# GeoStat-Framework/PyKrige

Measured on AMD Instinct MI355X. Metric: kriged grid-points/sec (z + sigma^2), OK2D N=5000 on 1000x1000 grid, higher is better.
Workload: dtype f64

## Files before the change

### include/mikrige.h

```cpp
#ifndef MIKRIGE_H
#define MIKRIGE_H
#include <stdint.h>
#ifdef __cplusplus
extern "C" {
#endif

#define MIK_ABI_VERSION 9

#define MIK_OK          0
#define MIK_EINVAL     (-1)
#define MIK_ESINGULAR  (-2)
#define MIK_EHIP       (-3)
#define MIK_ERCCL      (-4)
#define MIK_ESTATE     (-5)

#define MIK_MODEL_LINEAR      0
#define MIK_MODEL_POWER       1
#define MIK_MODEL_GAUSSIAN    2
#define MIK_MODEL_SPHERICAL   3
#define MIK_MODEL_EXPONENTIAL 4
#define MIK_MODEL_HOLE_EFFECT 5
#define MIK_MODEL_CUSTOM      6

typedef struct mik_handle mik_handle;
// ... 58 lines not shown
  int32_t mw_kernel;
  int32_t half_sweep;
  int32_t factor_attempts;
  int32_t null_dim;
  int32_t rhs_overlapped;
  double verify_ms;
  double verify_res_z;
  double verify_res_inv;
  int32_t sparse;
  int32_t stations_sorted;
  double sparse_tiles;
  double sparse_tiles_dense;
  double sparse_ktiles;
  double sparse_ktiles_dense;
  double sparse_lists_ms;
  double sparse_diag_products;
  int32_t sparse_rows;
  int32_t points_sorted;
  double sort_points_ms;
  int32_t sparse_ktile;
  int32_t reserved2;
  double exchange_bytes;
} mik_timing;

int  mik_device_count(void);
int  mik_abi_version(void);
int  mik_create(int device, mik_handle **out);
void mik_destroy(mik_handle *h);

int  mik_set_devices(int n);
int  mik_handle_set_devices(mik_handle *h, int n);
int  mik_handle_devices(mik_handle *h);
int  mik_slab_of(int64_t n, int members, int i, int64_t *lo, int64_t *count);

int  mik_set_option(mik_handle *h, const char *key, double value);

typedef void (*mik_variogram_fn)(void *user, double *d_inout, int64_t rows, int64_t cols, int64_t ld);
int  mik_set_custom_variogram(mik_handle *h, mik_variogram_fn fn, void *user);

int  mik_set_problem(mik_handle *h, const mik_problem *p);
int  mik_station_order(const mik_problem *p, int32_t *order_out);
int  mik_factor(mik_handle *h);
int  mik_set_points(mik_handle *h, const mik_points *g);
int  mik_set_grid(mik_handle *h, const mik_grid *g);
int  mik_adjust_points(mik_handle *h, const double center[3], const double rot[9], const double stretch[3]);
int  mik_predict(mik_handle *h);
int  mik_get_results(mik_handle *h, double *z_out, double *ss_out);
int  mik_take_results(mik_handle *h, double **z, double **ss);
void mik_release_results(double *z);

int  mik_set_fields(mik_handle *h, const double *values, int64_t n, int32_t nf);
int  mik_get_field_results(mik_handle *h, double *z_out);

int  mik_set_field_gaps(mik_handle *h, const uint8_t *valid , int64_t n, int32_t nf);
int  mik_get_field_sigmasq(mik_handle *h, double *ss_out);
int  mik_synchronize(mik_handle *h);

int  mik_predict_moving_window(mik_handle *h, int n_closest_points);

int  mik_cross_validate(mik_handle *h, int n_closest_points , double *zhat_out , double *ss_out );

int  mik_cross_validate_folds(mik_handle *h, const int32_t *fold , int nfolds, double *zhat_out , double *ss_out );

int  mik_cross_validate_window(mik_handle *h, int n_closest_points, double *zhat_out , double *ss_out );

int  mik_predict_cov(mik_handle *h, double *cov_out );
// ... 39 lines not shown
```

### pykrige_amd/_lib.py

```python
import ctypes as C
import os

import numpy as np

_HERE = os.path.dirname(os.path.abspath(__file__))
LIB_PATH = os.environ.get("MIK_LIB_PATH") or os.path.join(_HERE, "libmikrige.so")

MIK_OK, MIK_EINVAL, MIK_ESINGULAR, MIK_EHIP, MIK_ERCCL, MIK_ESTATE = 0, -1, -2, -3, -4, -5
MODEL_IDS = {"linear": 0, "power": 1, "gaussian": 2, "spherical": 3, "exponential": 4, "hole-effect": 5, "custom": 6}
VARIOGRAM_FN = C.CFUNCTYPE(None, C.c_void_p, C.POINTER(C.c_double), C.c_int64, C.c_int64, C.c_int64)

_dp = C.POINTER(C.c_double)


class MikProblem(C.Structure):
    _fields_ = [
        ("ndim", C.c_int32), ("model_id", C.c_int32), ("n", C.c_int64),
        ("xs", _dp), ("ys", _dp), ("zs", _dp), ("values", _dp),
        ("params", C.c_double * 3), ("eps", C.c_double),
        ("exact_values", C.c_int32), ("regional_linear", C.c_int32), ("n_wells", C.c_int32), ("n_extra", C.c_int32),
        ("wells", _dp), ("extra_cols", _dp), ("a_inv", _dp),
        ("geographic", C.c_int32), ("pseudo_inv", C.c_int32),
    ]

# ... 19 lines not shown
    _fields_ = [
        ("assemble_ms", C.c_double), ("invert_ms", C.c_double), ("rhs_ms", C.c_double),
        ("contract_ms", C.c_double), ("predict_ms", C.c_double), ("contract_launches", C.c_int64),
        ("contract_flops_executed", C.c_double), ("factor_path", C.c_int32), ("symmetric", C.c_int32),
        ("engine", C.c_int32), ("reserved", C.c_int32),
        ("exchange_ms", C.c_double), ("exchange_path", C.c_int32), ("n_devices", C.c_int32),
        ("exchange_wait_ms", C.c_double), ("exchange_fallbacks", C.c_int32), ("rccl_ranks", C.c_int32),
        ("mw_kernel", C.c_int32), ("half_sweep", C.c_int32), ("factor_attempts", C.c_int32), ("null_dim", C.c_int32), ("rhs_overlapped", C.c_int32),
        ("verify_ms", C.c_double), ("verify_res_z", C.c_double), ("verify_res_inv", C.c_double),
        ("sparse", C.c_int32), ("stations_sorted", C.c_int32),
        ("sparse_tiles", C.c_double), ("sparse_tiles_dense", C.c_double),
        ("sparse_ktiles", C.c_double), ("sparse_ktiles_dense", C.c_double), ("sparse_lists_ms", C.c_double),
        ("sparse_diag_products", C.c_double), ("sparse_rows", C.c_int32), ("points_sorted", C.c_int32),
        ("sort_points_ms", C.c_double), ("sparse_ktile", C.c_int32), ("reserved2", C.c_int32), ("exchange_bytes", C.c_double),
    ]

    def as_dict(self):
        return {k: getattr(self, k) for k, _ in self._fields_}


_lib = None
ABI_VERSION = 9
CV_FOLDS_LDS = 96

SIGNATURES = {
    "mik_device_count": (C.c_int, []),
    "mik_abi_version": (C.c_int, []),
    "mik_create": (C.c_int, [C.c_int, C.POINTER(C.c_void_p)]),
    "mik_destroy": (None, [C.c_void_p]),
    "mik_set_devices": (C.c_int, [C.c_int]),
    "mik_handle_set_devices": (C.c_int, [C.c_void_p, C.c_int]),
    "mik_handle_devices": (C.c_int, [C.c_void_p]),
    "mik_slab_of": (C.c_int, [C.c_int64, C.c_int, C.c_int, C.POINTER(C.c_int64), C.POINTER(C.c_int64)]),
    "mik_get_device_timing": (C.c_int, [C.c_void_p, C.c_int, C.POINTER(MikTiming)]),
    "mik_set_option": (C.c_int, [C.c_void_p, C.c_char_p, C.c_double]),
    "mik_set_problem": (C.c_int, [C.c_void_p, C.POINTER(MikProblem)]),
    "mik_station_order": (C.c_int, [C.POINTER(MikProblem), C.POINTER(C.c_int32)]),
    "mik_factor": (C.c_int, [C.c_void_p]),
    "mik_set_points": (C.c_int, [C.c_void_p, C.POINTER(MikPoints)]),
    "mik_set_grid": (C.c_int, [C.c_void_p, C.POINTER(MikGrid)]),
    "mik_adjust_points": (C.c_int, [C.c_void_p, _dp, _dp, _dp]),
    "mik_predict": (C.c_int, [C.c_void_p]),
    "mik_get_results": (C.c_int, [C.c_void_p, _dp, _dp]),
    "mik_take_results": (C.c_int, [C.c_void_p, C.POINTER(_dp), C.POINTER(_dp)]),
    "mik_release_results": (None, [_dp]),
    "mik_set_fields": (C.c_int, [C.c_void_p, _dp, C.c_int64, C.c_int32]),
    "mik_get_field_results": (C.c_int, [C.c_void_p, _dp]),
    "mik_set_field_gaps": (C.c_int, [C.c_void_p, C.POINTER(C.c_uint8), C.c_int64, C.c_int32]),
    "mik_get_field_sigmasq": (C.c_int, [C.c_void_p, _dp]),
    "mik_synchronize": (C.c_int, [C.c_void_p]),
    "mik_set_custom_variogram": (C.c_int, [C.c_void_p, VARIOGRAM_FN, C.c_void_p]),
    "mik_predict_cov": (C.c_int, [C.c_void_p, _dp]),
    "mik_predict_block": (C.c_int, [C.c_void_p, _dp, C.c_int]),
    "mik_predict_block_window": (C.c_int, [C.c_void_p, _dp, C.c_int, C.c_int]),
    "mik_predict_moving_window": (C.c_int, [C.c_void_p, C.c_int]),
    "mik_predict_window_gaps": (C.c_int, [C.c_void_p, C.c_int, C.POINTER(C.c_uint8), _dp, _dp]),
    "mik_cross_validate": (C.c_int, [C.c_void_p, C.c_int, _dp, _dp]),
    "mik_cross_validate_folds": (C.c_int, [C.c_void_p, C.POINTER(C.c_int32), C.c_int, _dp, _dp]),
    "mik_cross_validate_window": (C.c_int, [C.c_void_p, C.c_int, _dp, _dp]),
    "mik_statistics": (C.c_int, [C.c_void_p, _dp, _dp]),
    "mik_experimental_variogram": (C.c_int, [C.c_void_p, C.c_int, _dp, _dp, C.POINTER(C.c_int32)]),
    "mik_krige_execute": (C.c_int, [C.c_int, C.POINTER(MikProblem), C.POINTER(MikPoints), _dp, _dp]),
    "mik_assemble_only": (C.c_int, [C.c_void_p]),
    "mik_get_matrix": (C.c_int, [C.c_void_p, C.c_int, _dp]),
    "mik_matrix_order": (C.c_int64, [C.c_void_p]),
    "mik_points_resident": (C.c_int64, [C.c_void_p]),
# ... 390 lines not shown
        self.option_epoch += 1
        check(self._lib.mik_comm_init(self._h, int(nranks), int(rank), C.create_string_buffer(uid, 128)))

    def bcast_factor(self, root=0):
        check(self._lib.mik_bcast_factor(self._h, int(root)))

    def factor_checksum(self):
        out = (C.c_uint64 * 4)()
        check(self._lib.mik_factor_checksum(self._h, out))
        return tuple(int(v) for v in out)

    def exchange_note(self):
        return (self._lib.mik_exchange_note(self._h) or b"").decode("utf-8", "replace")


def station_order(xs, ys, zs=None, geographic=False):
    xs, ys = _f64(xs), _f64(ys)
    zs = _f64(zs) if zs is not None else None
    p = MikProblem()
    p.ndim, p.n = (3 if zs is not None else 2), xs.size
    p.geographic = 1 if geographic else 0
    p.xs, p.ys, p.zs = _ptr(xs), _ptr(ys), _ptr(zs)
    out = np.zeros(xs.size, dtype=np.int32)
    check(load().mik_station_order(C.byref(p), out.ctypes.data_as(C.POINTER(C.c_int32))))
    return out


def slab_of(n, members, i):
    lo, cnt = C.c_int64(0), C.c_int64(0)
    check(load().mik_slab_of(int(n), int(members), int(i), C.byref(lo), C.byref(cnt)))
    return lo.value, cnt.value


def set_devices(n):
    flush_handle_pool()
    check(load().mik_set_devices(int(n)))


import threading as _threading

_pool_lock = _threading.Lock()
_pool = []


def _env_sig():
    return tuple(sorted((k, v) for k, v in os.environ.items() if k.startswith("MIK_") or k == "LOCAL_RANK"))


def acquire_handle():
    sig, pid = _env_sig(), os.getpid()
    with _pool_lock:
        for i, h in enumerate(_pool):
            if h.pid == pid and h.env_sig == sig:
                return _pool.pop(i)
    return Handle()


def release_handle(h, device_bytes):
    if h is None or not getattr(h, "_h", None):
        return
    try:
        limit = int(os.environ.get("MIK_HANDLE_POOL", "4"))
        cap = float(os.environ.get("MIK_HANDLE_POOL_BYTES", str(512 * 2 ** 20)))
    except ValueError:
        limit, cap = 0, 0.0
    if limit > 0 and h.option_epoch == 0 and getattr(h, "_custom_cb", None) is None and h.pid == os.getpid() and device_bytes <= cap:
# ... 39 lines not shown
```

### pykrige_amd/csrc/mik_host.h

```cpp
#pragma once
#include "mik_dev.h"
#include "../../include/mikrige.h"

#include <dlfcn.h>
#include <rccl/rccl.h>

#include <algorithm>
#include <array>
#include <cmath>
#include <cstdio>
#include <cstdlib>
#include <cstring>
#include <atomic>
#include <chrono>
#include <condition_variable>
#include <memory>
#include <map>
#include <mutex>
#include <string>
#include <thread>
#include <vector>

using namespace mik;

// ... 100 lines not shown
inline void host_copy(void* dst, const void* src, size_t bytes) {
  constexpr size_t PIECE = 8u << 20;
  const size_t nthr = std::min<size_t>(4, bytes / PIECE);
  if (nthr < 2) {
    memcpy(dst, src, bytes);
    return;
  }
  std::vector<std::thread> th;
  const size_t per = ((bytes / nthr + 63) / 64) * 64;
  for (size_t t = 1; t < nthr; ++t) {
    const size_t off = t * per, len = (t + 1 == nthr) ? bytes - off : per;
    th.emplace_back([=] { memcpy((char*)dst + off, (const char*)src + off, len); });
  }
  memcpy(dst, src, per);
  for (auto& t : th) t.join();
}

extern "C++" {
template <class F>
inline void parallel_chunks(long n, F fn) {
  const long nthr = std::min<long>(8, n / (1L << 20));
  if (nthr < 2) {
    fn(0, 0L, n);
    return;
  }
  std::vector<std::thread> th;
  const long per = (n + nthr - 1) / nthr;
  for (long t = 1; t < nthr; ++t) th.emplace_back([=] { fn((int)t, t * per, std::min(n, (t + 1) * per)); });
  fn(0, 0L, std::min(n, per));
  for (auto& t : th) t.join();
}
}
inline int chunks_of(long n) { return (int)std::max<long>(1, std::min<long>(8, n / (1L << 20))); }

inline void unmasked_positions(const int8_t* mask, long ncells, std::vector<long>& idx) {
  const int nc = chunks_of(ncells);
  std::vector<long> cnt(nc + 1, 0);
  parallel_chunks(ncells, [&](int c, long b, long e) {
    long k = 0;
    for (long i = b; i < e; ++i) k += mask[i] == 0;
    cnt[c + 1] = k;
  });
  for (int c = 0; c < nc; ++c) cnt[c + 1] += cnt[c];
  idx.resize((size_t)cnt[nc]);
  parallel_chunks(ncells, [&](int c, long b, long e) {
    long k = cnt[c];
    for (long i = b; i < e; ++i)
      if (!mask[i]) idx[(size_t)k++] = i;
  });
}

struct RcclApi {
  void* lib = nullptr;
  ncclResult_t (*GetUniqueId)(ncclUniqueId*) = nullptr;
  ncclResult_t (*CommInitRank)(ncclComm_t*, int, ncclUniqueId, int) = nullptr;
  ncclResult_t (*Broadcast)(const void*, void*, size_t, ncclDataType_t, int, ncclComm_t, hipStream_t) = nullptr;
  ncclResult_t (*CommDestroy)(ncclComm_t) = nullptr;
  const char* (*GetErrorString)(ncclResult_t) = nullptr;
  ncclResult_t (*CommInitAll)(ncclComm_t*, int, const int*) = nullptr;
  ncclResult_t (*GroupStart)() = nullptr;
  ncclResult_t (*GroupEnd)() = nullptr;
};
inline RcclApi g_rccl;
inline int rccl_load() {
  if (g_rccl.lib) return MIK_OK;
  const char* names[] = {getenv("MIK_RCCL_LIB") ? getenv("MIK_RCCL_LIB") : "librccl.so", "librccl.so", "librccl.so.1", "/opt/rocm/lib/librccl.so"};
// ... 102 lines not shown
  DevBuf Averify, vbuf;
  std::vector<double> hvals;
  int nf = 0;
  std::vector<double> hfields;
  DevBuf fv, fc, zf;
  PinBuf pin_fz;
  int fv_sorted = -1;
  int nf_done = 0;
  std::vector<uint8_t> hgaps;
  bool gaps_any = false;
  DevBuf gap_W, gap_work, gap_list, gap_part, gap_ss;
  PinBuf pin_gss;
  std::vector<int> gap_plane;
  PinBuf pin_cov;
  hipEvent_t ev_cov[6] = {nullptr, nullptr, nullptr, nullptr, nullptr, nullptr};
  int opt_gate = -1;
  int opt_panel_stream = -1;
  int opt_update_rev = -1;
  long npt_total = 0, npt = 0;
  bool masked = false;
  std::vector<long> scatter;
  const unsigned* scatter32 = nullptr;
  DevBuf mask_dev, mask_cnt;
  PinBuf scatter_pin;
  DevBuf px, py, pz, extra_rows, z, ss;
  DevBuf grid_axes, grid_idx;
  DevBuf mw_idx, mw_dist, stat_S, stat_x, stat_out;
  DevBuf cvw;
  int n_cu = 256;
  int t_state = 0;
  int opt_tri = 1;
  int opt_symmetrize = 1;
  int opt_factor = 0, opt_sym = 1;
  long opt_chunk = 131072;
  int opt_mw_pivot = 0;
  bool mw_force_piv = false;
  int opt_mw_lds_cap = 8192;
  int opt_mw_knn_bound = 1;
  int opt_mw_static = 1;
  int opt_mw_knn_lane = 1;
  int opt_mw_class = 0;
  mik_timing tm{};
  std::vector<hipEvent_t> evpool;
  std::vector<LaunchEvents> pr_launch;
  hipEvent_t ev_predict0 = nullptr, ev_predict1 = nullptr;
  hipEvent_t ev_lane1 = nullptr;
  hipEvent_t ev_sort = nullptr;
  hipEvent_t ev_chunk = nullptr;
  ncclComm_t comm = nullptr;
  int nranks = 1, rank = 0;
  PinBuf pin_in, pin_out;
  hipStream_t stream_d2h = nullptr;
  hipEvent_t ev_d2h = nullptr;
  bool results_on_host = false;
  long out_off = 0;
  std::vector<mik_handle*> kids;
  bool is_kid = false;
  bool alias_ok = false;
  int opt_exchange = 0;
  int exchange_used = 0;
  double exchange_ms = 0.0;
  std::string exchange_note;
  std::vector<std::vector<hipStream_t>> xstreams;
  std::vector<hipEvent_t> xevents;
  std::shared_ptr<struct XchgJob> xjob;
  hipStream_t xstream = nullptr;
  DevBuf xsum;
// ... 127 lines not shown
```

### pykrige_amd/csrc/mik_predict.hip

```cpp
#include "mik_k_predict.h"
#include "mik_k_cov.h"
#include "mik_host.h"

static int geo_point_vectors(mik_handle* h) {
  const long npt = h->npt;
  MIKC(h->gu.ensure(sizeof(double) * 3 * (size_t)npt));
  double* u = h->gu.as<double>();
  hipLaunchKernelGGL(k_geo_unit_p, dim3((unsigned)((npt + 255) / 256)), dim3(256), 0, h->stream, (const double*)h->px.as<double>(),
                     (const double*)h->py.as<double>(), npt, u, u + npt, u + 2 * npt);
  return MIK_OK;
}

int sort_points(mik_handle* h, long chunk, long nchunks) {
  const long npt = h->npt;
  const int kd = h->ndim;
  const int bits = ps_bits(kd), bps = (int)((chunk + MIK_PS_TILE - 1) / MIK_PS_TILE);
  for (int q = 0; q < 2; ++q) {
    MIKC(h->ps_key[q].ensure(sizeof(unsigned) * (size_t)npt));
    MIKC(h->ps_idx[q].ensure(sizeof(unsigned) * (size_t)npt));
  }
  MIKC(h->ps_table.ensure(sizeof(unsigned) * (size_t)nchunks * (1u << MIK_PS_DB) * (size_t)bps));
  MIKC(h->ps_box.ensure(sizeof(double) * 4 * (size_t)nchunks));
  const double *px = h->px.as<double>(), *py = h->py.as<double>(), *pz = h->ndim == 3 ? h->pz.as<double>() : nullptr;
  hipStream_t st = h->stream;
// ... 154 lines not shown
    HIPC(hipFuncSetAttribute((const void*)k_cv_folds<MIK_FB, false>, hipFuncAttributeMaxDynamicSharedMemorySize, (int)lds));
    hipLaunchKernelGGL((k_cv_folds<MIK_FB, false>), dim3((unsigned)nsmall), dim3(256), lds, h->stream, a);
  }
  if (nbig) {
    const size_t lds = sizeof(double) * 2 * MIK_CVF_NB * MIK_CVF_TLD;
    a.desc += 3 * (size_t)nsmall;
    HIPC(hipFuncSetAttribute((const void*)k_cv_folds<MIK_FB, true>, hipFuncAttributeMaxDynamicSharedMemorySize, (int)lds));
    hipLaunchKernelGGL((k_cv_folds<MIK_FB, true>), dim3((unsigned)nbig), dim3(256), lds, h->stream, a);
  }
  HIPC(hipGetLastError());
  return cv_copy_back(h, a.zhat, a.ss, nf, sorted, zhat_out, ss_out);
}

static constexpr int SP_GROUP = 16;

struct Plan {
  long npt, chunk, nchunks;
  int Mp, nIblk, nK16, nKt, kend, nf;
  bool sparse, gathered, sortpts, lanes2;
  const unsigned* perm;
  bool gaps;
  int gap_np, gap_nRblk;
  const long* gap_desc;
  double* panel;
};

struct Launch {
  long c, t0;
  int nvalid, palloc, nTb;
  Launch(const Plan& p, long c_)
      : c(c_), t0(c_ * p.chunk), nvalid((int)std::min<long>(p.chunk, p.npt - t0)), palloc(((nvalid + 127) / 128) * 128), nTb(palloc / 128) {}
};

static int plan_predict(mik_handle* h, Plan& p, bool cov) {
  const long npt = h->npt;
  const int Mp = h->Mp, nIblk = Mp / 128, nf = h->nf;
  p.npt = npt, p.Mp = Mp, p.nIblk = nIblk, p.nK16 = Mp / 16, p.nf = nf;
  p.kend = ((h->M + MIK_BK - 1) / MIK_BK) * MIK_BK;
  if (nf > 1) {
    MIKC(h->zf.ensure(sizeof(double) * (size_t)(nf - 1) * (size_t)npt));
    HIPC(hipEventSynchronize(h->ev_d2h));
    MIKC(h->pin_fz.ensure(sizeof(double) * (size_t)(nf - 1) * (size_t)npt));
  }
  if (nf > 0 && h->gaps_any) HIPC(hipEventSynchronize(h->ev_d2h));
  long chunk = std::min<long>(h->opt_chunk, ((npt + 127) / 128) * 128);
  if (h->model == MIK_MODEL_CUSTOM) chunk = std::min<long>(chunk, 16384);
  p.gaps = nf > 0 && h->gaps_any;
  p.sparse = h->factor_sorted && h->opt_sparse != 2 && h->opt_sparse != 0 && !p.gaps;
  const bool shared_panel = cov && !p.sparse;
  if (p.sparse) chunk = std::min<long>(chunk, 131072);
  p.gathered = p.sparse && h->opt_sparse_rows != 128 && (double)Mp * (double)Mp * 8.0 < 4294967296.0;
  p.nKt = p.gathered ? Mp / 8 : p.nK16;
  h->tm.sparse_ktile = !p.sparse ? 0 : p.gathered ? 8 : 16;
  h->tm.sparse = p.sparse ? 1 : 0;
  h->tm.sparse_rows = p.sparse ? (p.gathered ? 16 : 128) : 0;
  h->tm.stations_sorted = h->factor_sorted ? 1 : 0;
  h->tm.sparse_tiles = h->tm.sparse_tiles_dense = h->tm.sparse_ktiles = h->tm.sparse_ktiles_dense = h->tm.sparse_lists_ms = 0.0;
  h->tm.sparse_diag_products = 0.0;
  p.sortpts = p.sparse && (h->opt_sort_points == 1 || (h->opt_sort_points < 0 && npt >= 4096 && Mp >= 512));
  h->tm.points_sorted = p.sortpts ? 1 : 0;
  h->tm.sort_points_ms = 0.0;
  const bool lanes2_wanted = p.sparse && h->opt_sparse_lanes == 2;
  size_t freeb = 0, totalb = 0;
  HIPC(hipMemGetInfo(&freeb, &totalb));
  const size_t have = h->lane[0].Bt.bytes + h->lane[1].Bt.bytes;
  while (!shared_panel && chunk > 128 && (size_t)chunk * Mp * sizeof(double) * (lanes2_wanted ? 2 : 1) > std::max(freeb + have, have) / 2) chunk = ((chunk / 2 + 127) / 128) * 128;
  long nchunks = (npt + chunk - 1) / chunk;
  chunk = (((npt + nchunks - 1) / nchunks + 127) / 128) * 128;
  nchunks = (npt + chunk - 1) / chunk;
  p.chunk = chunk, p.nchunks = nchunks;
  p.lanes2 = lanes2_wanted && nchunks > 1;
  MIKC(h->pin_out.ensure(sizeof(double) * 2 * (size_t)npt));
  if ((long)h->pr_launch.size() < nchunks) h->pr_launch.resize((size_t)nchunks);
  for (LaunchEvents& ev : h->pr_launch)
    for (hipEvent_t* e : ev.all())
      if (!*e) HIPC(hipEventCreate(e));
  const size_t nTb = (size_t)chunk / 128;
  for (int L = 0; L < (p.lanes2 ? 2 : 1); ++L) {
    PredictLane& ln = h->lane[L];
    if (!shared_panel) MIKC(ln.Bt.ensure(sizeof(double) * (size_t)chunk * Mp));
    MIKC(ln.part.ensure(sizeof(double) * (size_t)chunk * nIblk));
    MIKC(ln.queue.ensure(8 * sizeof(unsigned long long)));
    if (!p.sparse) break;
    MIKC(ln.cand.ensure(nTb * p.nK16));
    MIKC(ln.flags.ensure(nTb * p.nKt));
    MIKC(ln.klist.ensure(sizeof(unsigned short) * nTb * p.nKt));
    MIKC(ln.kcount.ensure(sizeof(int) * nTb));
    MIKC(ln.nrows.ensure(sizeof(int) * nTb));
    if (p.gathered) {
      MIKC(ln.recs.ensure(48 * nTb * nIblk));
    } else {
      MIKC(ln.rows.ensure(sizeof(unsigned short) * nTb * nIblk));
      MIKC(ln.rstart.ensure(sizeof(unsigned short) * nTb * nIblk));
      MIKC(ln.tiles.ensure(sizeof(unsigned) * nTb * nIblk));
    }
    MIKC(ln.xoff.ensure(sizeof(int) * 9));
  }
  if (p.sparse) MIKC(h->sp_stats.ensure(sizeof(unsigned long long) * 4 * (size_t)nchunks));
  return MIK_OK;
}

static RhsArgs rhs_args(mik_handle* h, const Plan& p, const Launch& l) {
// ... 344 lines not shown
    ga.xoff = ln.xoff.as<int>();
    ga.queue = ln.queue.as<unsigned long long>();
    static const bool spg_prof = getenv("MIK_SPG_PROF") && atoi(getenv("MIK_SPG_PROF")) != 0;
    if (spg_prof) MIKC(spg_profile(ga, nb, sc));
    else hipLaunchKernelGGL((k_contract_spg<2, true, true>), dim3(nb), dim3(512), 0, sc, ga);
  } else {
    SpArgs sa{};
    sa.Ainv = h->T.as<double>();
    sa.lda = p.Mp;
    sa.Bt = ln.Bt.as<double>();
    sa.ldb = p.Mp;
    sa.part = ln.part.as<double>();
    sa.palloc = l.palloc;
    sa.kend = p.kend;
    sa.nIblk = nIblk;
    sa.nK16 = p.nK16;
    sa.klist = ln.klist.as<unsigned short>();
    sa.kcount = ln.kcount.as<int>();
    sa.rows = ln.rows.as<unsigned short>();
    sa.rstart = ln.rstart.as<unsigned short>();
    sa.tiles = ln.tiles.as<unsigned>();
    sa.xoff = ln.xoff.as<int>();
    sa.queue = ln.queue.as<unsigned long long>();
    hipLaunchKernelGGL((k_contract_sp<2>), dim3(nb), dim3(512), 0, sc, sa);
  }
  HIPC(hipEventRecord(ev.contract_end, sc));
  hipLaunchKernelGGL(k_ss_reduce_sp, dim3((l.nvalid + 255) / 256), dim3(256), 0, sc, (const double*)ln.part.as<double>(), l.palloc,
                     (const int*)ln.nrows.as<int>(), l.nvalid, 2.0 * (h->v.p0 + h->v.p2),
                     p.perm ? h->ss.as<double>() : h->ss.as<double>() + l.t0, p.perm ? p.perm + l.t0 : (const unsigned*)nullptr);
  if (p.lanes2 && (l.c & 1)) HIPC(hipEventRecord(h->ev_lane1, sc));
  return MIK_OK;
}

static int copy_out(mik_handle* h, const Plan& p, const Launch& l, hipStream_t st) {
  const size_t bytes = sizeof(double) * l.nvalid;
  HIPC(hipEventRecord(h->ev_chunk, st));
  HIPC(hipStreamWaitEvent(h->stream_d2h, h->ev_chunk, 0));
  HIPC(hipMemcpyAsync(h->pin_out.as<double>() + l.t0, h->z.as<double>() + l.t0, bytes, hipMemcpyDeviceToHost, h->stream_d2h));
  HIPC(hipMemcpyAsync(h->pin_out.as<double>() + p.npt + l.t0, h->ss.as<double>() + l.t0, bytes, hipMemcpyDeviceToHost, h->stream_d2h));
  for (int f = 1; f < p.nf; ++f)
    HIPC(hipMemcpyAsync(h->pin_fz.as<double>() + (size_t)(f - 1) * p.npt + l.t0, h->zf.as<double>() + (size_t)(f - 1) * p.npt + l.t0, bytes,
                        hipMemcpyDeviceToHost, h->stream_d2h));
  for (int q = 0; q < (p.gaps ? p.gap_np : 0); ++q)
    HIPC(hipMemcpyAsync(h->pin_gss.as<double>() + (size_t)q * p.npt + l.t0, h->gap_ss.as<double>() + (size_t)q * p.npt + l.t0, bytes,
                        hipMemcpyDeviceToHost, h->stream_d2h));
  return MIK_OK;
}

static int read_back(mik_handle* h, const Plan& p, bool sorted_now) {
  float ms = 0.f;
  HIPC(hipEventElapsedTime(&ms, h->ev_predict0, h->ev_predict1));
  h->tm.predict_ms = ms;
  if (sorted_now) {
    HIPC(hipEventElapsedTime(&ms, h->ev_predict0, h->ev_sort));
    h->tm.sort_points_ms = ms;
  }
  std::vector<unsigned long long> sp(p.sparse ? 4 * (size_t)p.nchunks : 0);
  if (p.sparse) HIPC(hipMemcpy(sp.data(), h->sp_stats.p, sizeof(unsigned long long) * sp.size(), hipMemcpyDeviceToHost));
  const bool tri = h->opt_sym && h->opt_tri;
  double kext = 0.0;
  for (int ib = 0; ib < p.nIblk; ++ib) {
    const int ext = h->opt_sym ? std::max(0, p.kend - ib * 128) : p.kend;
    if (tri) {
      const int nt = std::min(ext, 128) / 16;
      kext += (ext - 16 * nt) + 16.0 * (nt * (nt + 1) / 2) / 8.0;
    } else kext += ext;
  }
  const int ntl = (p.kend - (p.nIblk - 1) * 128) / 16;
  for (long c = 0; c < p.nchunks; ++c) {
    const LaunchEvents& ev = h->pr_launch[(size_t)c];
    const int nTb = Launch(p, c).nTb;
    HIPC(hipEventElapsedTime(&ms, ev.rhs_begin, ev.rhs_end));
    h->tm.rhs_ms += ms;
    HIPC(hipEventElapsedTime(&ms, ev.contract_begin, ev.contract_end));
    h->tm.contract_ms += ms;
// ... 63 lines not shown
  }
  if (prof) {
    float m0 = 0.f, m1 = 0.f, m2 = 0.f;
    HIPC(hipEventElapsedTime(&m0, h->ev_cov[0], h->ev_cov[1]));
    HIPC(hipEventElapsedTime(&m1, h->ev_cov[1], h->ev_cov[2]));
    HIPC(hipEventElapsedTime(&m2, h->ev_cov[2], h->ev_cov[3]));
    const double mc = std::chrono::duration<double, std::milli>(std::chrono::steady_clock::now() - t0).count();
    fprintf(stderr, "mik_predict_cov: P %ld Pp %ld Mp %d kend %d stage0_ms %.4f stage1_ms %.4f stage2_ms %.4f copy_ms %.4f\n", P, Pp, p.Mp, p.kend,
            m0, m1, m2, mc);
  }
  return MIK_OK;
}

static int predict_prologue(mik_handle* h, const char* who, bool* empty) {
  if (!h || !h->have_factor) return fail(MIK_ESTATE, std::string(who) + ": factor first");
  if (!h->have_points) return fail(MIK_ESTATE, std::string(who) + ": set points first");
  HIPC(hipSetDevice(h->device));
  reset_predict_timing(h);
  h->tm.symmetric = h->opt_sym;
  h->tm.engine = 0;
  h->tm.mw_kernel = 0;
  h->nf_done = h->nf;
  h->gap_plane.clear();
  *empty = h->npt == 0;
  if (*empty) h->have_results = true;
  return MIK_OK;
}

static int predict_body(mik_handle* h, double* cov_out) {
  bool empty = false;
  MIKC(predict_prologue(h, "mik_predict", &empty));
  if (empty) return MIK_OK;
  Plan p{};
  MIKC(plan_predict(h, p, cov_out != nullptr));
  const long Pp = ((h->npt + 127) / 128) * 128;
  DevBuf cov_bt, cov_yt, cov_c, cov_z;
  if (cov_out) {
    MIKC(cov_bt.ensure(sizeof(double) * (size_t)Pp * (size_t)p.Mp));
    MIKC(cov_yt.ensure(sizeof(double) * (size_t)Pp * (size_t)p.Mp));
    MIKC(cov_c.ensure(sizeof(double) * (size_t)Pp * (size_t)Pp));
    if (!p.sparse) p.panel = cov_bt.as<double>();
  }
  HIPC(hipStreamWaitEvent(h->stream, h->ev_d2h, 0));
  if (p.sparse && h->geo) MIKC(geo_point_vectors(h));
  if (p.nf > 0) MIKC(fields_coefficients(h));
  HIPC(hipEventRecord(h->ev_predict0, h->stream));
  if (p.gaps) MIKC(gaps_setup(h, p));
  bool sorted_now = false;
  if (p.sortpts && !(h->ps_valid && h->ps_chunk == p.chunk)) {
    MIKC(sort_points(h, p.chunk, p.nchunks));
    HIPC(hipEventRecord(h->ev_sort, h->stream));
    sorted_now = true;
  }
  if (p.sortpts) p.perm = h->ps_idx[0].as<unsigned>();
  if (p.lanes2) HIPC(hipStreamWaitEvent(h->stream2, h->ev_predict0, 0));
  if (p.lanes2 && sorted_now) HIPC(hipStreamWaitEvent(h->stream2, h->ev_sort, 0));
  for (long c = 0; c < p.nchunks; ++c) {
    const Launch l(p, c);
    const int L = p.lanes2 ? (int)(c & 1) : 0;
    hipStream_t st = L ? h->stream2 : h->stream;
    MIKC(launch_rhs(h, p, l, h->lane[L], st));
    MIKC(p.sparse ? contract_sparse(h, p, l, h->lane[L], st) : contract_dense(h, p, l));
    MIKC(copy_out(h, p, l, st));
  }
  HIPC(hipGetLastError());
  if (p.lanes2) HIPC(hipStreamWaitEvent(h->stream, h->ev_lane1, 0));
  HIPC(hipEventRecord(h->ev_predict1, h->stream));
  HIPC(hipEventRecord(h->ev_d2h, h->stream_d2h));
  if (cov_out && p.sparse) {
    MIKC(cov_z.ensure(sizeof(double) * (size_t)Pp));
    Plan d = p;
    d.sparse = d.gathered = d.sortpts = d.lanes2 = false;
    d.perm = nullptr, d.nf = 0, d.panel = cov_bt.as<double>();
    for (long c = 0; c < d.nchunks; ++c) MIKC(launch_rhs(h, d, Launch(d, c), h->lane[0], h->stream, cov_z.as<double>()));
    p.panel = d.panel;
  }
  if (cov_out) MIKC(cov_stages(h, p, Pp, cov_yt.as<double>(), cov_c.as<double>(), cov_out));
  HIPC(hipStreamSynchronize(h->stream));
  MIKC(read_back(h, p, sorted_now));
  h->have_results = true;
  return MIK_OK;
}

int one_predict(mik_handle* h) { return predict_body(h, nullptr); }

int one_predict_cov(mik_handle* h, double* cov_out) { return predict_body(h, cov_out); }

#include "mik_k_block.h"

#define DISPATCH_BLOCK_NDIM(model, NDIM, KERNEL, grid, block, stream, args)                          \
  switch (model) {                                                                                   \
    case 0: hipLaunchKernelGGL((KERNEL<0, NDIM>), grid, block, 0, stream, args); break;              \
    case 1: hipLaunchKernelGGL((KERNEL<1, NDIM>), grid, block, 0, stream, args); break;              \
    case 2: hipLaunchKernelGGL((KERNEL<2, NDIM>), grid, block, 0, stream, args); break;              \
    case 3: hipLaunchKernelGGL((KERNEL<3, NDIM>), grid, block, 0, stream, args); break;              \
    case 4: hipLaunchKernelGGL((KERNEL<4, NDIM>), grid, block, 0, stream, args); break;              \
// ... 79 lines not shown
```

### pykrige_amd/csrc/mikrige.hip

```cpp
#include "mik_k_core.h"
#include "mik_host.h"

extern "C" {

const char* mik_last_error(void) { return g_err.c_str(); }

int mik_abi_version(void) { return MIK_ABI_VERSION; }

int mik_device_count(void) {
  int n = 0;
  if (hipGetDeviceCount(&n) != hipSuccess) return 0;
  return n;
}

static void destroy_one(mik_handle* h);

static double env_seconds(const char* name, double dflt) {
  const char* e = getenv(name);
  if (!e || !*e) return dflt;
  const double v = atof(e);
  return v > 0.0 ? v : dflt;
}

static int create_one_body(mik_handle* h, int device) {
// ... 129 lines not shown
    const int dev = i == 0 ? h->device : h->kids[i - 1]->device;
    (void)hipSetDevice(dev);
    for (hipStream_t st : h->xstreams[i])
      if (st) (void)hipStreamDestroy(st);
  }
  h->xstreams.clear();
  for (mik_handle* k : h->kids) destroy_one(k);
  h->kids.clear();
  (void)hipSetDevice(h->device);
}

static int set_group(mik_handle* h, int n) {
  if (h->is_kid) return fail(MIK_EINVAL, "mik_handle_set_devices: not on a member of a device group");
  int visible = 0;
  if (hipGetDeviceCount(&visible) != hipSuccess || visible <= 0) return fail(MIK_EHIP, "no HIP device visible");
  if (n == 0) n = visible;
  if (n < 1 || n > 64) return fail(MIK_EINVAL, "number of devices out of range");
  if (n > visible && !h->alias_ok)
    return fail(MIK_EINVAL, "more devices requested than are visible (option alias_devices / MIK_ALIAS_DEVICES=1 lets several "
                            "logical devices share one GPU -- for tests on a 1-GPU box)");
  if ((int)h->kids.size() + 1 == n) return MIK_OK;
  release_group(h);
  for (int i = 1; i < n; ++i) {
    mik_handle* k = nullptr;
    const int rc = create_one((h->device + i) % visible, &k);
    if (rc != MIK_OK) {
      const std::string keep = g_err;
      release_group(h);
      g_err = keep;
      return rc;
    }
    k->is_kid = true;
    k->opt_factor = h->opt_factor, k->opt_sym = h->opt_sym;
    k->opt_chunk = h->opt_chunk, k->opt_symsweep = h->opt_symsweep, k->opt_panel_stream = h->opt_panel_stream, k->opt_update_rev = h->opt_update_rev, k->opt_lookahead = h->opt_lookahead, k->opt_gate = h->opt_gate, k->opt_pinv_fast = h->opt_pinv_fast, k->opt_verify = h->opt_verify, k->verify_tol_z = h->verify_tol_z, k->verify_tol_inv = h->verify_tol_inv;
    k->opt_mw_class = h->opt_mw_class, k->opt_mw_knn_bound = h->opt_mw_knn_bound, k->opt_mw_pivot = h->opt_mw_pivot, k->opt_mw_lds_cap = h->opt_mw_lds_cap, k->opt_tri = h->opt_tri, k->opt_symmetrize = h->opt_symmetrize;
    k->opt_sparse = h->opt_sparse, k->opt_sparse_lanes = h->opt_sparse_lanes, k->opt_sparse_rows = h->opt_sparse_rows, k->opt_sort_points = h->opt_sort_points, k->opt_drift_eq = h->opt_drift_eq;
    k->opt_pinv_block = h->opt_pinv_block, k->opt_mw_static = h->opt_mw_static, k->opt_mw_knn_lane = h->opt_mw_knn_lane;
    k->custom_fn = h->custom_fn, k->custom_user = h->custom_user;
    h->kids.push_back(k);
  }
  h->have_problem = h->have_factor = h->have_points = h->have_results = false;
  h->t_state = 0;
  HIPC(hipSetDevice(h->device));
  return MIK_OK;
}

int mik_create(int device, mik_handle** out) {
  if (!out) return fail(MIK_EINVAL, "mik_create: out is NULL");
  mik_handle* h = nullptr;
  MIKC(create_one(device, &h));
  const int want = default_devices();
  if (want != 1) {
    int visible = 1;
    (void)hipGetDeviceCount(&visible);
    const int rc = set_group(h, want == 0 ? visible : want);
    if (rc != MIK_OK) {
      const std::string keep = g_err;
      destroy_one(h);
      g_err = keep;
      return rc;
    }
  }
  *out = h;
  return MIK_OK;
}

void mik_destroy(mik_handle* h) {
// ... 36 lines not shown
  } else if (!strcmp(key, "exchange")) {
    if (value < 0 || value > 3) return fail(MIK_EINVAL, "exchange must be 0 (auto), 1 (rccl), 2 (peer copies) or 3 (redundant factorisation)");
    h->opt_exchange = (int)value;
  } else if (!strcmp(key, "exchange_tri")) {
    h->opt_exchange_tri = value != 0.0;
  } else if (!strcmp(key, "alias_devices")) {
    h->alias_ok = value != 0.0;
  } else if (!strcmp(key, "factor")) {
    if (value < 0 || value > 2) return fail(MIK_EINVAL, "factor must be 0 (auto), 1 (sweep) or 2 (pivoted)");
    h->opt_factor = (int)value;
  } else if (!strcmp(key, "symmetric")) {
    h->opt_sym = value != 0.0;
  } else if (!strcmp(key, "sparse")) {
    if (value != -1.0 && value != 0.0 && value != 1.0 && value != 2.0) return fail(MIK_EINVAL, "sparse must be -1 (auto), 0, 1 or 2");
    h->opt_sparse = (int)value;
  } else if (!strcmp(key, "sort_points")) {
    if (value != -1.0 && value != 0.0 && value != 1.0) return fail(MIK_EINVAL, "sort_points must be -1 (auto), 0 or 1");
    h->opt_sort_points = (int)value;
  } else if (!strcmp(key, "sparse_rows")) {
    if (value != -1.0 && value != 16.0 && value != 128.0) return fail(MIK_EINVAL, "sparse_rows must be -1 (auto), 16 or 128");
    h->opt_sparse_rows = (int)value;
  } else if (!strcmp(key, "sparse_lanes")) {
    if (value != 1.0 && value != 2.0) return fail(MIK_EINVAL, "sparse_lanes must be 1 or 2");
    h->opt_sparse_lanes = (int)value;
  } else if (!strcmp(key, "drift_eq")) {
    h->opt_drift_eq = value != 0.0;
  } else if (!strcmp(key, "tri")) {
    h->opt_tri = value != 0.0;
  } else if (!strcmp(key, "symmetrize")) {
    h->opt_symmetrize = value != 0.0;
  } else if (!strcmp(key, "chunk")) {
    if (value < 128) return fail(MIK_EINVAL, "chunk must be >= 128");
    h->opt_chunk = ((long)value / 128) * 128;
  } else if (!strcmp(key, "symsweep")) {
    h->opt_symsweep = value < 0.0 ? -1 : (value != 0.0);
  } else if (!strcmp(key, "verify")) {
    h->opt_verify = value != 0.0;
  } else if (!strcmp(key, "verify_tol_z") || !strcmp(key, "verify_tol_inv")) {
    if (!(value > 0.0)) return fail(MIK_EINVAL, "a tolerance must be positive");
    (key[11] == 'z' ? h->verify_tol_z : h->verify_tol_inv) = value;
  } else if (!strcmp(key, "pinv_fast")) {
    h->opt_pinv_fast = value != 0.0;
  } else if (!strcmp(key, "pinv_block")) {
    h->opt_pinv_block = value < 0.0 ? -1 : (value != 0.0);
  } else if (!strcmp(key, "gate")) {
    h->opt_gate = value < 0.0 ? -1 : (value != 0.0);
  } else if (!strcmp(key, "update_rev")) {
    h->opt_update_rev = value < 0.0 ? -1 : value != 0.0 ? 1 : 0;
  } else if (!strcmp(key, "panel_stream")) {
    h->opt_panel_stream = value < 0.0 ? -1 : (value != 0.0);
  } else if (!strcmp(key, "lookahead")) {
    h->opt_lookahead = value < 0.0 ? -1 : (value != 0.0);
  } else if (!strcmp(key, "mw_knn_bound")) {
    h->opt_mw_knn_bound = value != 0.0;
  } else if (!strcmp(key, "mw_knn_lane")) {
    h->opt_mw_knn_lane = value != 0.0;
  } else if (!strcmp(key, "mw_static")) {
    h->opt_mw_static = value != 0.0;
  } else if (!strcmp(key, "mw_class")) {
    h->opt_mw_class = (int)value;
  } else if (!strcmp(key, "mw_pivot")) {
    h->opt_mw_pivot = value != 0.0;
  } else if (!strcmp(key, "mw_lds_cap")) {
    if (value < 0 || value > 8192) return fail(MIK_EINVAL, "mw_lds_cap must be in 0..8192");
    h->opt_mw_lds_cap = (int)value;
  } else {
// ... 906 lines not shown
      }
      for (int d = 0; d < h->ndim; ++d) h->pts_extent = std::max(h->pts_extent, ehi[d] - elo[d]);
      std::nth_element(st.begin(), st.begin() + ns / 2, st.end());
      h->pts_step = st[(size_t)(ns / 2)];
    }
  }
  h->have_points = true;
  h->points_from_grid = false;
  h->points_adjusted = false;
  h->ps_valid = false;
  h->have_results = false;
  return MIK_OK;
}

static void slab_of(long n, int members, int i, long* lo, long* cnt) {
  auto cut = [&](int k) {
    if (k >= members) return n;
    const long c = (long)((double)n * k / members);
    return std::min(n, (c / 128) * 128);
  };
  *lo = cut(i);
  *cnt = cut(i + 1) - *lo;
}

int mik_slab_of(int64_t n, int members, int i, int64_t* lo, int64_t* count) {
  if (n < 0 || members < 1 || i < 0 || i >= members || !lo || !count) return fail(MIK_EINVAL, "mik_slab_of: bad argument");
  long l, c;
  slab_of((long)n, members, i, &l, &c);
  *lo = l;
  *count = c;
  return MIK_OK;
}

int mik_set_points(mik_handle* h, const mik_points* g) {
  if (!h || !g) return fail(MIK_EINVAL, "mik_set_points: NULL argument");
  if (!h->have_problem) return fail(MIK_ESTATE, "mik_set_points: set the problem first");
  if (g->npt < 0) return fail(MIK_EINVAL, "npt < 0");
  if (g->npt > 0 && (!g->px || !g->py || (h->ndim == 3 && !g->pz))) return fail(MIK_EINVAL, "point arrays missing");
  if (h->nextra > 0 && g->npt > 0 && !g->extra_rows) return fail(MIK_EINVAL, "extra_rows missing for host-evaluated drifts");
  h->npt_total = g->npt;
  std::vector<long> idx;
  long n = g->npt;
  h->masked = false;
  if (g->mask) {
    unmasked_positions(g->mask, g->npt, idx);
    n = (long)idx.size();
    h->masked = n != g->npt;
  }
  const long* ip = h->masked ? idx.data() : nullptr;
  const int members = (int)h->kids.size() + 1;
  return for_each_device(h, [&](int i, mik_handle* d) {
    long lo, cnt;
    slab_of(n, members, i, &lo, &cnt);
    return one_set_points(d, g, ip, lo, cnt);
  });
}

static int one_set_grid(mik_handle* h, bool leader, const mik_grid* g, const unsigned* idx, long lo, long n, long first, long ncells) {
  HIPC(hipSetDevice(h->device));
  HIPC(hipStreamSynchronize(h->stream_d2h));
  h->npt = n;
  h->out_off = lo;
  h->scatter.clear();
  h->scatter32 = idx ? idx + lo : nullptr;
  const long cap = std::max<long>(n, 1);
  const int three = g->ndim == 3;
// ... 894 lines not shown
```

### pykrige_amd/kriging.py

```python
import contextlib
import os as _os
import warnings

import numpy as np

from . import _lib
from . import core
from . import variogram_models


@contextlib.contextmanager
def _singular_as(backend):
    try:
        yield
    except np.linalg.LinAlgError as e:
        if backend == "C":
            raise ValueError("Singular matrix") from e
        raise


class _Cols:

    __slots__ = ("cols", "shape")

# ... 179 lines not shown
        elif variogram_model not in core.MODELS:
            raise ValueError("Specified variogram model '%s' is not supported." % variogram_model)
        else:
            self.variogram_function = self.variogram_dict[variogram_model]
        self.variogram_model = variogram_model
        if getattr(self, "coordinates_type", "euclidean") == "geographic":
            if anisotropy.get("anisotropy_scaling", 1.0) != 1.0 and anisotropy["anisotropy_scaling"] != self.anisotropy_scaling:
                warnings.warn("Anisotropy is not compatible with geographic coordinates. Ignoring user set anisotropy.",
                              UserWarning)
        elif any(v != getattr(self, k) for k, v in anisotropy.items()):
            if self.verbose:
                print("Adjusting data for anisotropy...")
            for k, v in anisotropy.items():
                setattr(self, k, v)
            self._adjust_stations()
        self._set_variogram_parameters(variogram_parameters, nlags, weight, updating=True)

    def update_variogram_model(self, variogram_model, variogram_parameters=None, variogram_function=None, nlags=6,
                               weight=False, anisotropy_scaling=1.0, anisotropy_angle=0.0):
        self._update_variogram_model(variogram_model, variogram_parameters, variogram_function, nlags, weight,
                                     dict(anisotropy_scaling=anisotropy_scaling, anisotropy_angle=anisotropy_angle))

    def _get_handle(self):
        if self._handle is None:
            self._handle = _lib.acquire_handle()
        return self._handle

    _max_points = 0
    _max_fields = 0

    def _handle_bytes(self):
        n = int(np.size(self._values())) + 16
        mp = -(-n // 128) * 128
        npt = min(int(self._max_points), 131072)
        nf = self._max_fields + 16
        return 8.0 * (3.0 * mp * mp + 2.0 * npt * mp + 8.0 * self._max_points + 8.0 * n
                      + (nf * (mp + n + self._max_points) if self._max_fields else 0.0))

    def __getstate__(self):
        state = dict(self.__dict__)
        state["_handle"] = None
        state.pop("_factor_key", None)
        return state

    def __del__(self):
        h = self.__dict__.get("_handle")
        if h is not None:
            self._handle = None
            try:
                _lib.release_handle(h, self._handle_bytes())
            except Exception:
                pass

    def _values(self):
        return self.VALUES if self._ndim == 3 else self.Z

    def _station_extra_cols(self):
        return None

    def _wells(self):
        return None

    def _regional_linear(self):
        return False

    def _set_problem(self, h, with_drift=True, values=None, pseudo_inv=False, exact_values=None, eps=None):
        self._factor_key = None
# ... 1314 lines not shown
```

Baseline: 2.749 million.

## Size dense prediction chunks from free memory and copy z before contraction

When no chunk size is set, the dense prediction planner now picks the chunk from a memory budget (half of free device memory plus buffers already held), so a whole grid may run in one or a few launches instead of fixed 131072-point chunks. The z result is copied to the host right after the RHS step, so that transfer overlaps the sigma-squared contraction. This cuts launch and per-chunk overhead. In exchange it needs much larger B-tile buffers and raises the pool memory estimate, which risks memory pressure and less overlap between chunks.

```diff
diff --git a/include/mikrige.h b/include/mikrige.h
--- a/include/mikrige.h
+++ b/include/mikrige.h
@@ -114,6 +114,7 @@
 int  mik_handle_set_devices(mik_handle *h, int n);
 int  mik_handle_devices(mik_handle *h);
 int  mik_slab_of(int64_t n, int members, int i, int64_t *lo, int64_t *count);
+int  mik_dense_plan(int64_t npt, int mp, double budget_bytes, int64_t out[4]);
 
 int  mik_set_option(mik_handle *h, const char *key, double value);
 
diff --git a/pykrige_amd/_lib.py b/pykrige_amd/_lib.py
--- a/pykrige_amd/_lib.py
+++ b/pykrige_amd/_lib.py
@@ -75,6 +75,7 @@
     "mik_handle_set_devices": (C.c_int, [C.c_void_p, C.c_int]),
     "mik_handle_devices": (C.c_int, [C.c_void_p]),
     "mik_slab_of": (C.c_int, [C.c_int64, C.c_int, C.c_int, C.POINTER(C.c_int64), C.POINTER(C.c_int64)]),
+    "mik_dense_plan": (C.c_int, [C.c_int64, C.c_int, C.c_double, C.POINTER(C.c_int64)]),
     "mik_get_device_timing": (C.c_int, [C.c_void_p, C.c_int, C.POINTER(MikTiming)]),
     "mik_set_option": (C.c_int, [C.c_void_p, C.c_char_p, C.c_double]),
     "mik_set_problem": (C.c_int, [C.c_void_p, C.POINTER(MikProblem)]),
@@ -531,6 +532,12 @@
     return lo.value, cnt.value
 
 
+def dense_plan(npt, mp, budget_bytes):
+    out = (C.c_int64 * 4)()
+    check(load().mik_dense_plan(int(npt), int(mp), float(budget_bytes), out))
+    return tuple(int(v) for v in out)
+
+
 def set_devices(n):
     flush_handle_pool()
     check(load().mik_set_devices(int(n)))
diff --git a/pykrige_amd/csrc/mik_host.h b/pykrige_amd/csrc/mik_host.h
--- a/pykrige_amd/csrc/mik_host.h
+++ b/pykrige_amd/csrc/mik_host.h
@@ -156,6 +156,17 @@
 }
 }
 inline int chunks_of(long n) { return (int)std::max<long>(1, std::min<long>(8, n / (1L << 20))); }
+
+inline void dense_launch_shape(long npt, long Mp, double budget, long* chunk, long* nchunks) {
+  const double per_point = 8.0 * (double)(Mp + Mp / 128);
+  const long all = ((npt + 127) / 128) * 128;
+  const double fit = budget / per_point;
+  long c = fit >= (double)all ? all : std::max<long>(128, ((long)fit / 128) * 128);
+  long n = (npt + c - 1) / c;
+  c = (((npt + n - 1) / n + 127) / 128) * 128;
+  n = (npt + c - 1) / c;
+  *chunk = c, *nchunks = n;
+}
 
 inline void unmasked_positions(const int8_t* mask, long ncells, std::vector<long>& idx) {
   const int nc = chunks_of(ncells);
@@ -324,7 +335,8 @@
   int opt_tri = 1;
   int opt_symmetrize = 1;
   int opt_factor = 0, opt_sym = 1;
-  long opt_chunk = 131072;
+  long opt_chunk = 0;
+  double opt_plan_budget = 0.0;
   int opt_mw_pivot = 0;
   bool mw_force_piv = false;
   int opt_mw_lds_cap = 8192;
diff --git a/pykrige_amd/csrc/mik_predict.hip b/pykrige_amd/csrc/mik_predict.hip
--- a/pykrige_amd/csrc/mik_predict.hip
+++ b/pykrige_amd/csrc/mik_predict.hip
@@ -210,7 +210,7 @@
       : c(c_), t0(c_ * p.chunk), nvalid((int)std::min<long>(p.chunk, p.npt - t0)), palloc(((nvalid + 127) / 128) * 128), nTb(palloc / 128) {}
 };
 
-static int plan_predict(mik_handle* h, Plan& p, bool cov) {
+static int plan_predict(mik_handle* h, Plan& p, bool cov, bool whole = false) {
   const long npt = h->npt;
   const int Mp = h->Mp, nIblk = Mp / 128, nf = h->nf;
   p.npt = npt, p.Mp = Mp, p.nIblk = nIblk, p.nK16 = Mp / 16, p.nf = nf;
@@ -221,7 +221,7 @@
     MIKC(h->pin_fz.ensure(sizeof(double) * (size_t)(nf - 1) * (size_t)npt));
   }
   if (nf > 0 && h->gaps_any) HIPC(hipEventSynchronize(h->ev_d2h));
-  long chunk = std::min<long>(h->opt_chunk, ((npt + 127) / 128) * 128);
+  long chunk = std::min<long>(h->opt_chunk ? h->opt_chunk : 131072L, ((npt + 127) / 128) * 128);
   if (h->model == MIK_MODEL_CUSTOM) chunk = std::min<long>(chunk, 16384);
   p.gaps = nf > 0 && h->gaps_any;
   p.sparse = h->factor_sorted && h->opt_sparse != 2 && h->opt_sparse != 0 && !p.gaps;
@@ -246,6 +246,10 @@
   long nchunks = (npt + chunk - 1) / chunk;
   chunk = (((npt + nchunks - 1) / nchunks + 127) / 128) * 128;
   nchunks = (npt + chunk - 1) / chunk;
+  if (whole && !p.sparse && !p.gaps && !shared_panel && nf <= 1 && h->opt_chunk == 0 && h->model != MIK_MODEL_CUSTOM) {
+    const size_t held = h->lane[0].Bt.bytes + h->lane[0].part.bytes;
+    dense_launch_shape(npt, Mp, h->opt_plan_budget > 0.0 ? h->opt_plan_budget : (double)(std::max(freeb + held, held) / 2), &chunk, &nchunks);
+  }
   p.chunk = chunk, p.nchunks = nchunks;
   p.lanes2 = lanes2_wanted && nchunks > 1;
   MIKC(h->pin_out.ensure(sizeof(double) * 2 * (size_t)npt));
@@ -656,15 +660,19 @@
   return MIK_OK;
 }
 
-static int copy_out(mik_handle* h, const Plan& p, const Launch& l, hipStream_t st) {
+enum { COPY_Z = 1, COPY_SS = 2 };
+static int copy_out(mik_handle* h, const Plan& p, const Launch& l, hipStream_t st, int what = COPY_Z | COPY_SS) {
   const size_t bytes = sizeof(double) * l.nvalid;
   HIPC(hipEventRecord(h->ev_chunk, st));
   HIPC(hipStreamWaitEvent(h->stream_d2h, h->ev_chunk, 0));
-  HIPC(hipMemcpyAsync(h->pin_out.as<double>() + l.t0, h->z.as<double>() + l.t0, bytes, hipMemcpyDeviceToHost, h->stream_d2h));
+  if (what & COPY_Z) {
+    HIPC(hipMemcpyAsync(h->pin_out.as<double>() + l.t0, h->z.as<double>() + l.t0, bytes, hipMemcpyDeviceToHost, h->stream_d2h));
+    for (int f = 1; f < p.nf; ++f)
+      HIPC(hipMemcpyAsync(h->pin_fz.as<double>() + (size_t)(f - 1) * p.npt + l.t0, h->zf.as<double>() + (size_t)(f - 1) * p.npt + l.t0, bytes,
+                          hipMemcpyDeviceToHost, h->stream_d2h));
+  }
+  if (!(what & COPY_SS)) return MIK_OK;
   HIPC(hipMemcpyAsync(h->pin_out.as<double>() + p.npt + l.t0, h->ss.as<double>() + l.t0, bytes, hipMemcpyDeviceToHost, h->stream_d2h));
-  for (int f = 1; f < p.nf; ++f)
-    HIPC(hipMemcpyAsync(h->pin_fz.as<double>() + (size_t)(f - 1) * p.npt + l.t0, h->zf.as<double>() + (size_t)(f - 1) * p.npt + l.t0, bytes,
-                        hipMemcpyDeviceToHost, h->stream_d2h));
   for (int q = 0; q < (p.gaps ? p.gap_np : 0); ++q)
     HIPC(hipMemcpyAsync(h->pin_gss.as<double>() + (size_t)q * p.npt + l.t0, h->gap_ss.as<double>() + (size_t)q * p.npt + l.t0, bytes,
                         hipMemcpyDeviceToHost, h->stream_d2h));
@@ -794,7 +802,7 @@
   MIKC(predict_prologue(h, "mik_predict", &empty));
   if (empty) return MIK_OK;
   Plan p{};
-  MIKC(plan_predict(h, p, cov_out != nullptr));
+  MIKC(plan_predict(h, p, cov_out != nullptr, cov_out == nullptr));
   const long Pp = ((h->npt + 127) / 128) * 128;
   DevBuf cov_bt, cov_yt, cov_c, cov_z;
   if (cov_out) {
@@ -822,8 +830,9 @@
     const int L = p.lanes2 ? (int)(c & 1) : 0;
     hipStream_t st = L ? h->stream2 : h->stream;
     MIKC(launch_rhs(h, p, l, h->lane[L], st));
+    if (!p.sparse) MIKC(copy_out(h, p, l, st, COPY_Z));
     MIKC(p.sparse ? contract_sparse(h, p, l, h->lane[L], st) : contract_dense(h, p, l));
-    MIKC(copy_out(h, p, l, st));
+    MIKC(copy_out(h, p, l, st, p.sparse ? COPY_Z | COPY_SS : COPY_SS));
   }
   HIPC(hipGetLastError());
   if (p.lanes2) HIPC(hipStreamWaitEvent(h->stream, h->ev_lane1, 0));
diff --git a/pykrige_amd/csrc/mikrige.hip b/pykrige_amd/csrc/mikrige.hip
--- a/pykrige_amd/csrc/mikrige.hip
+++ b/pykrige_amd/csrc/mikrige.hip
@@ -185,7 +185,7 @@
     }
     k->is_kid = true;
     k->opt_factor = h->opt_factor, k->opt_sym = h->opt_sym;
-    k->opt_chunk = h->opt_chunk, k->opt_symsweep = h->opt_symsweep, k->opt_panel_stream = h->opt_panel_stream, k->opt_update_rev = h->opt_update_rev, k->opt_lookahead = h->opt_lookahead, k->opt_gate = h->opt_gate, k->opt_pinv_fast = h->opt_pinv_fast, k->opt_verify = h->opt_verify, k->verify_tol_z = h->verify_tol_z, k->verify_tol_inv = h->verify_tol_inv;
+    k->opt_chunk = h->opt_chunk, k->opt_plan_budget = h->opt_plan_budget, k->opt_symsweep = h->opt_symsweep, k->opt_panel_stream = h->opt_panel_stream, k->opt_update_rev = h->opt_update_rev, k->opt_lookahead = h->opt_lookahead, k->opt_gate = h->opt_gate, k->opt_pinv_fast = h->opt_pinv_fast, k->opt_verify = h->opt_verify, k->verify_tol_z = h->verify_tol_z, k->verify_tol_inv = h->verify_tol_inv;
     k->opt_mw_class = h->opt_mw_class, k->opt_mw_knn_bound = h->opt_mw_knn_bound, k->opt_mw_pivot = h->opt_mw_pivot, k->opt_mw_lds_cap = h->opt_mw_lds_cap, k->opt_tri = h->opt_tri, k->opt_symmetrize = h->opt_symmetrize;
     k->opt_sparse = h->opt_sparse, k->opt_sparse_lanes = h->opt_sparse_lanes, k->opt_sparse_rows = h->opt_sparse_rows, k->opt_sort_points = h->opt_sort_points, k->opt_drift_eq = h->opt_drift_eq;
     k->opt_pinv_block = h->opt_pinv_block, k->opt_mw_static = h->opt_mw_static, k->opt_mw_knn_lane = h->opt_mw_knn_lane;
@@ -288,6 +288,8 @@
   } else if (!strcmp(key, "chunk")) {
     if (value < 128) return fail(MIK_EINVAL, "chunk must be >= 128");
     h->opt_chunk = ((long)value / 128) * 128;
+  } else if (!strcmp(key, "plan_budget")) {
+    h->opt_plan_budget = value;
   } else if (!strcmp(key, "symsweep")) {
     h->opt_symsweep = value < 0.0 ? -1 : (value != 0.0);
   } else if (!strcmp(key, "verify")) {
@@ -1260,6 +1262,14 @@
   return MIK_OK;
 }
 
+int mik_dense_plan(int64_t npt, int mp, double budget_bytes, int64_t out[4]) {
+  if (npt < 1 || mp < 128 || mp % 128 || !(budget_bytes >= 0.0) || !out) return fail(MIK_EINVAL, "mik_dense_plan: bad argument");
+  long chunk, n;
+  dense_launch_shape((long)npt, mp, budget_bytes, &chunk, &n);
+  out[0] = chunk, out[1] = n, out[2] = 8 * chunk * (int64_t)mp, out[3] = 8 * chunk * (int64_t)(mp / 128);
+  return MIK_OK;
+}
+
 int mik_set_points(mik_handle* h, const mik_points* g) {
   if (!h || !g) return fail(MIK_EINVAL, "mik_set_points: NULL argument");
   if (!h->have_problem) return fail(MIK_ESTATE, "mik_set_points: set the problem first");
diff --git a/pykrige_amd/kriging.py b/pykrige_amd/kriging.py
--- a/pykrige_amd/kriging.py
+++ b/pykrige_amd/kriging.py
@@ -235,7 +235,7 @@
     def _handle_bytes(self):
         n = int(np.size(self._values())) + 16
         mp = -(-n // 128) * 128
-        npt = min(int(self._max_points), 131072)
+        npt = int(self._max_points)
         nf = self._max_fields + 16
         return 8.0 * (3.0 * mp * mp + 2.0 * npt * mp + 8.0 * self._max_points + 8.0 * n
                       + (nf * (mp + n + self._max_points) if self._max_fields else 0.0))
```

Result: no change. 2.760 million (median of 6 runs) (+0.4%).
